# 86885974647565434342125458569795756674/torch.distributed.pipeline.sync.Pipe

Hardware: AMD Instinct MI355X
Metric: tokens/sec for 12-layer Transformer at PP=N (pipeline-parallel training) (higher is better)
Workload: dtype bf16

## Files before the change

mipipe/csrc/bindings.cpp:

```cpp
#include <torch/extension.h>
#include <ATen/hip/HIPContext.h>
#include <ATen/hip/HIPGeneratorImpl.h>
#include <ATen/core/Generator.h>
#include <ATen/hip/impl/HIPGuardImplMasqueradingAsCUDA.h>
#include <ATen/hip/impl/HIPStreamMasqueradingAsCUDA.h>

#include <mutex>
#include <optional>
#include <tuple>

#include "kernels/kernels.h"
#include "runtime/ipc.h"
#include "runtime/runtime.h"

namespace py = pybind11;
using at::Tensor;

namespace mipipe {
namespace {

#define MP_CHECK(cond, ...) TORCH_CHECK(cond, "mipipe: ", __VA_ARGS__)

hipStream_t cur_stream(const Tensor& t) { return at::hip::getCurrentHIPStreamMasqueradingAsCUDA(t.device().index()).stream(); }

// ... 1126 lines not shown
  m.def("attention_supported", [](int64_t S, int64_t D) { return attention_supported((int)S, (int)D); });
  m.def("attention_f32_supported", [](int64_t S, int64_t D) { return attention_f32_supported((int)S, (int)D); });
  m.def("attention_fwd", &py_attention_fwd, py::arg("q"), py::arg("k"), py::arg("v"), py::arg("causal"), py::arg("p"),
        py::arg("scale"), py::arg("kv_len") = 0, py::arg("words") = py::none(), py::arg("words_seed") = 0,
        py::arg("words_offset") = 0);
  m.def("attention_bwd", &py_attention_bwd, py::arg("dout"), py::arg("q"), py::arg("k"), py::arg("v"), py::arg("o"),
        py::arg("lse"), py::arg("causal"), py::arg("p"), py::arg("scale"), py::arg("seed"), py::arg("offset"),
        py::arg("dq"), py::arg("dk"), py::arg("dv"), py::arg("bits") = py::none(), py::arg("kv_len") = 0);
  m.def("attention_long_supported", [](int64_t S, int64_t D) { return attention_long_supported((int)S, (int)D); });
  m.def("attention_long_set_fused_rng", &attention_long_set_fused_rng,
        "long-sequence attention: make the dropout keep words inside the forward kernel (true, default) or in a "
        "kernel of their own before it (false)");
  m.def("gemm_supported", &py_gemm_supported);
  m.def("gemm_f32_supported", &py_gemm_f32_supported);
  m.def("attention_set_fused_bwd", &attention_set_fused_bwd);
  m.def("gemm_set_schedule", &gemm_set_schedule,
        "256x256 GEMM main loop: 7 whole-tile ping-pong (default, the only one in the product build); a "
        "--gemm-ab build also has the A/B schedules 0-6 (kernels.h).  Returns false for a schedule not built in.");
  m.def("gemm_get_schedule", &gemm_get_schedule);
  m.def("gemm_ab_build", &gemm_ab_build, "true if the A/B GEMM schedules 0-6 are compiled in (-DMIPIPE_GEMM_AB)");
  m.def("gemm_set_rounds", &gemm_set_rounds,
        "multi-round GEMM grids whose last round is at most half full: 0 one launch, 1 (default) one launch per round "
        "of tiles when K >= 4096, 2 one launch per round at any K");
  m.def("gemm_set_splitk", &gemm_set_splitk, "split-K factor of under-filled long-K GEMMs: 0 off, 1 auto (default), n >= 2 forced");
  m.def("gemm_set_waves", &gemm_set_waves,
        "256x256 GEMM blocks: 4 = one wave per SIMD with a 128x128 tile each (gemm4w_kernel), 8 = the ping-pong kernel, "
        "0 = default");
  m.def("gemm_get_waves", &gemm_get_waves);
  m.def("gemm_set_width", &gemm_set_width, "256-row GEMM block width: 0 auto (grid-quantisation rule), 128, 256");
  m.def("linear_fwd", &py_linear_fwd, py::arg("x"), py::arg("w"), py::arg("bias"), py::arg("act"), py::arg("p"),
// ... 29 lines not shown
```

mipipe/csrc/kernels/attention.hip:

```cpp
#include "common.h"
#include "kernels.h"

namespace mipipe {

namespace {

typedef __attribute__((ext_vector_type(4))) short s16x4;
typedef __attribute__((ext_vector_type(8))) short s16x8;
typedef __attribute__((address_space(3))) s16x4 lds_s16x4;

constexpr int kRows = 64;
constexpr int kThreads = 256;
constexpr float kLog2e = 1.4426950408889634f;

template <int D>
struct Img {
  static constexpr int kRowBytes = 2 * D;
  static constexpr int kChunks = D / 8;
  static constexpr int kBytes = kRows * kRowBytes;
  __device__ static __forceinline__ int f(int r) {
    if constexpr (kChunks >= 16) return (((r ^ (r >> 2)) & 1) << 1) | ((r & 2) << 1) | (r & 8);
    else if constexpr (kChunks == 8) return ((((r >> 1) ^ (r >> 2)) & 1) << 1) | ((r >> 1) & 4);
    else return (((r & 3) << 2) | ((r >> 2) & 3)) & (kChunks - 1);
  }
// ... 822 lines not shown
    }
}

namespace shortseq {

constexpr int S = 128;
constexpr int kThreads = 512;
constexpr int kChunk = 64;
constexpr int kChunkImg = S * kChunk * 2;
constexpr int kSqImg = S * S * 2;
constexpr int kStageBytes = 3 * kChunkImg;
constexpr int kPOff = 4 * kChunkImg;
constexpr int kDsOff = kPOff + kSqImg;
constexpr int kSmem = kDsOff + kSqImg;
constexpr int kFwdPOff = 2 * kChunkImg;
constexpr int kFwdSmem = kFwdPOff + kSqImg;

__device__ __forceinline__ int coff(int r, int c16) { return Img<64>::off(r, c16); }
__device__ __forceinline__ int soff(int r, int c16) { return Img<128>::off(r, c16); }

__device__ __forceinline__ void load_chunk(const bf16_t* __restrict__ base, int64_t ld, int d0, int tid, uint4& v0,
                                           uint4& v1) {
  const int r = tid >> 3, c = tid & 7;
  v0 = *reinterpret_cast<const uint4*>(base + (int64_t)r * ld + d0 + 8 * c);
  v1 = *reinterpret_cast<const uint4*>(base + (int64_t)(r + 64) * ld + d0 + 8 * c);
}
__device__ __forceinline__ void store_chunk(char* img, int tid, const uint4& v0, const uint4& v1) {
  const int r = tid >> 3, c = tid & 7;
  *reinterpret_cast<uint4*>(img + coff(r, c)) = v0;
  *reinterpret_cast<uint4*>(img + coff(r + 64, c)) = v1;
}

__device__ __forceinline__ bf16x8 crow(const char* img, int rb, int s, int lane) {
  return *reinterpret_cast<const bf16x8*>(img + coff(rb + (lane & 15), 4 * s + (lane >> 4)));
}
__device__ __forceinline__ bf16x8 ccol(const char* img, int db, int s, int lane) {
  const int g = lane >> 4, q = (lane & 15) >> 2, p = lane & 3;
  const int r0 = 32 * s + 8 * g + q;
  const int c8 = (db >> 2) + p;
  const int o0 = coff(r0, c8 >> 1) + 8 * (c8 & 1);
  const int o1 = coff(r0 + 4, c8 >> 1) + 8 * (c8 & 1);
  const s16x4 lo = __builtin_amdgcn_ds_read_tr16_b64_v4i16((lds_s16x4*)(img + o0));
  const s16x4 hi = __builtin_amdgcn_ds_read_tr16_b64_v4i16((lds_s16x4*)(img + o1));
  return __builtin_bit_cast(bf16x8, __builtin_shufflevector(lo, hi, 0, 1, 2, 3, 4, 5, 6, 7));
}
__device__ __forceinline__ bf16x8 srow(const char* img, int rb, int s, int lane) {
  return *reinterpret_cast<const bf16x8*>(img + soff(rb + (lane & 15), 4 * s + (lane >> 4)));
}
__device__ __forceinline__ bf16x8 scol(const char* img, int ib, int s, int lane) {
  const int g = lane >> 4, q = (lane & 15) >> 2, p = lane & 3;
  const int r0 = 32 * s + 8 * g + q;
  const int c8 = (ib >> 2) + p;
  const int o0 = soff(r0, c8 >> 1) + 8 * (c8 & 1);
  const int o1 = soff(r0 + 4, c8 >> 1) + 8 * (c8 & 1);
  const s16x4 lo = __builtin_amdgcn_ds_read_tr16_b64_v4i16((lds_s16x4*)(img + o0));
  const s16x4 hi = __builtin_amdgcn_ds_read_tr16_b64_v4i16((lds_s16x4*)(img + o1));
  return __builtin_bit_cast(bf16x8, __builtin_shufflevector(lo, hi, 0, 1, 2, 3, 4, 5, 6, 7));
}

template <int D, bool CAUSAL>
__global__ void __launch_bounds__(kThreads, 1) attn_bwd_s128_kernel(AttnArgs a) {
  extern __shared__ __attribute__((aligned(16))) char smem[];
  const int tid = threadIdx.x, lane = tid & 63, wave = __builtin_amdgcn_readfirstlane(tid >> 6);
  const int bh = blockIdx.x;
  const int b = bh / a.H, h = bh % a.H;
  const int64_t boff = (int64_t)b * a.sb_qkv + (int64_t)h * a.sh_qkv;
  const bf16_t* Q = reinterpret_cast<const bf16_t*>(a.q) + boff;
  const bf16_t* K = reinterpret_cast<const bf16_t*>(a.k) + boff;
  const bf16_t* V = reinterpret_cast<const bf16_t*>(a.v) + boff;
  const bf16_t* dO = reinterpret_cast<const bf16_t*>(a.dout) + (int64_t)b * a.sb_o + (int64_t)h * a.sh_o;
  constexpr int NC = D / kChunk;

  f32x4 sacc[8], pacc[8];
#pragma unroll
  for (int j = 0; j < 8; ++j) sacc[j] = pacc[j] = f32x4{0.f, 0.f, 0.f, 0.f};
  const int myrow = wave * 16 + (lane & 15);
  const bf16_t* qrow = Q + (int64_t)myrow * a.ld_qkv;
  const bf16_t* drow = dO + (int64_t)myrow * a.ld_o;

  uint4 k0, k1, v0, v1;
  load_chunk(K, a.ld_qkv, 0, tid, k0, k1);
  load_chunk(V, a.ld_qkv, 0, tid, v0, v1);
  store_chunk(smem, tid, k0, k1);
  store_chunk(smem + kChunkImg, tid, v0, v1);
  __syncthreads();
#pragma unroll 1
  for (int c = 0; c < NC; ++c) {
    const char* kimg = smem + (c & 1) * 2 * kChunkImg;
    const char* vimg = kimg + kChunkImg;
    if (c + 1 < NC) {
      load_chunk(K, a.ld_qkv, (c + 1) * kChunk, tid, k0, k1);
      load_chunk(V, a.ld_qkv, (c + 1) * kChunk, tid, v0, v1);
    }
    bf16x8 qf[2], df[2];
#pragma unroll
    for (int s2 = 0; s2 < 2; ++s2) {
      qf[s2] = frag_global(qrow + c * kChunk, s2, lane);
      df[s2] = frag_global(drow + c * kChunk, s2, lane);
    }
#pragma unroll
    for (int s2 = 0; s2 < 2; ++s2)
#pragma unroll
      for (int j = 0; j < 8; ++j) {
        sacc[j] = __builtin_amdgcn_mfma_f32_16x16x32_bf16(qf[s2], crow(kimg, 16 * j, s2, lane), sacc[j], 0, 0, 0);
        pacc[j] = __builtin_amdgcn_mfma_f32_16x16x32_bf16(df[s2], crow(vimg, 16 * j, s2, lane), pacc[j], 0, 0, 0);
      }
    if (c + 1 < NC) {
      char* nimg = smem + ((c + 1) & 1) * 2 * kChunkImg;
      store_chunk(nimg, tid, k0, k1);
      store_chunk(nimg + kChunkImg, tid, v0, v1);
    }
    __syncthreads();
  }

  const int qrow0 = wave * 16 + 4 * (lane >> 4);
  const float sl2 = a.scale * kLog2e;
  const float pscale = a.p > 0.f ? 1.f / (1.f - a.p) : 1.f;
  float lse2[4];
#pragma unroll
  for (int r = 0; r < 4; ++r) lse2[r] = a.lse[(int64_t)bh * S + qrow0 + r] * kLog2e;
  float dsum[4] = {0.f, 0.f, 0.f, 0.f};
#pragma unroll
  for (int j = 0; j < 8; ++j) {
    const int key = 16 * j + (lane & 15);
    uint32_t w[4] = {0xFFFFFFFFu, 0xFFFFFFFFu, 0xFFFFFFFFu, 0xFFFFFFFFu};
    if (a.p > 0.f) {
      const uint4 mw = attn_mask_words(a, bh, qrow0 >> 2, key);
      w[0] = mw.x; w[1] = mw.y; w[2] = mw.z; w[3] = mw.w;
    }
#pragma unroll
    for (int r = 0; r < 4; ++r) {
      float pr = __builtin_amdgcn_exp2f(sacc[j][r] * sl2 - lse2[r]);
      if (CAUSAL && key > qrow0 + r) pr = 0.f;
      float dp = pacc[j][r];
      float pd = pr;
      if (a.p > 0.f) {
        const bool keep = w[r] >= a.threshold;
        dp = keep ? dp * pscale : 0.f;
        pd = keep ? pr * pscale : 0.f;
      }
      sacc[j][r] = pr;
      pacc[j][r] = dp;
      dsum[r] += pr * dp;
      *reinterpret_cast<bf16_t*>(smem + kPOff + soff(qrow0 + r, key >> 3) + 2 * (key & 7)) = f2bf(pd);
    }
  }
  float delta[4];
#pragma unroll
  for (int r = 0; r < 4; ++r) delta[r] = row_reduce_sum16(dsum[r]);
#pragma unroll
  for (int j = 0; j < 8; ++j) {
    const int key = 16 * j + (lane & 15);
#pragma unroll
    for (int r = 0; r < 4; ++r) {
      const float ds = sacc[j][r] * (pacc[j][r] - delta[r]);
      *reinterpret_cast<bf16_t*>(smem + kDsOff + soff(qrow0 + r, key >> 3) + 2 * (key & 7)) = f2bf(ds);
    }
  }

  const char* pimg = smem + kPOff;
  const char* dsimg = smem + kDsOff;
  char* kimg = smem;
  char* qimg = smem + kChunkImg;
  char* dimg = smem + 2 * kChunkImg;
  bf16_t* dQ = reinterpret_cast<bf16_t*>(a.dq) + boff;
  bf16_t* dK = reinterpret_cast<bf16_t*>(a.dk) + boff;
  bf16_t* dV = reinterpret_cast<bf16_t*>(a.dv) + boff;
  const int r0 = wave * 16;
  uint4 a0, a1, b0, b1, e0, e1;
  load_chunk(K, a.ld_qkv, 0, tid, a0, a1);
  load_chunk(Q, a.ld_qkv, 0, tid, b0, b1);
  load_chunk(dO, a.ld_o, 0, tid, e0, e1);
#pragma unroll 1
  for (int c = 0; c < NC; ++c) {
    const int d0 = c * kChunk;
    __syncthreads();
    store_chunk(kimg, tid, a0, a1);
    store_chunk(qimg, tid, b0, b1);
    store_chunk(dimg, tid, e0, e1);
    __syncthreads();
    if (c + 1 < NC) {
      load_chunk(K, a.ld_qkv, d0 + kChunk, tid, a0, a1);
      load_chunk(Q, a.ld_qkv, d0 + kChunk, tid, b0, b1);
      load_chunk(dO, a.ld_o, d0 + kChunk, tid, e0, e1);
    }
    f32x4 dq[4], dk[4], dv[4];
#pragma unroll
    for (int t = 0; t < 4; ++t) dq[t] = dk[t] = dv[t] = f32x4{0.f, 0.f, 0.f, 0.f};
#pragma unroll
    for (int ks = 0; ks < 4; ++ks) {
      const bf16x8 a_dq = srow(dsimg, r0, ks, lane);
      const bf16x8 a_dk = scol(dsimg, r0, ks, lane);
      const bf16x8 a_dv = scol(pimg, r0, ks, lane);
#pragma unroll
      for (int t = 0; t < 4; ++t) {
        dq[t] = __builtin_amdgcn_mfma_f32_16x16x32_bf16(a_dq, ccol(kimg, 16 * t, ks, lane), dq[t], 0, 0, 0);
        dk[t] = __builtin_amdgcn_mfma_f32_16x16x32_bf16(a_dk, ccol(qimg, 16 * t, ks, lane), dk[t], 0, 0, 0);
        dv[t] = __builtin_amdgcn_mfma_f32_16x16x32_bf16(a_dv, ccol(dimg, 16 * t, ks, lane), dv[t], 0, 0, 0);
      }
    }
    const int orow = r0 + 4 * (lane >> 4);
    __syncthreads();
#pragma unroll
    for (int t = 0; t < 4; ++t) {
      const int col = 16 * t + (lane & 15);
#pragma unroll
      for (int r = 0; r < 4; ++r) {
        const int at = coff(orow + r, col >> 3) + 2 * (col & 7);
        *reinterpret_cast<bf16_t*>(kimg + at) = f2bf(dq[t][r] * a.scale);
        *reinterpret_cast<bf16_t*>(qimg + at) = f2bf(dk[t][r] * a.scale);
        *reinterpret_cast<bf16_t*>(dimg + at) = f2bf(dv[t][r]);
      }
    }
    __syncthreads();
    {
      const int r = tid >> 3, cc = tid & 7;
#pragma unroll
      for (int h2 = 0; h2 < 2; ++h2) {
        const int row = r + 64 * h2;
        const int off = coff(row, cc);
        const int64_t g = (int64_t)row * a.ld_qkv + d0 + 8 * cc;
        *reinterpret_cast<uint4*>(dQ + g) = *reinterpret_cast<const uint4*>(kimg + off);
        *reinterpret_cast<uint4*>(dK + g) = *reinterpret_cast<const uint4*>(qimg + off);
        *reinterpret_cast<uint4*>(dV + g) = *reinterpret_cast<const uint4*>(dimg + off);
      }
    }
  }
}

template <int D, bool CAUSAL>
__global__ void __launch_bounds__(kThreads, 2) attn_fwd_s128_kernel(AttnArgs a) {
  extern __shared__ __attribute__((aligned(16))) char smem[];
  const int tid = threadIdx.x, lane = tid & 63, wave = __builtin_amdgcn_readfirstlane(tid >> 6);
  const int bh = blockIdx.x;
  const int b = bh / a.H, h = bh % a.H;
  const int64_t boff = (int64_t)b * a.sb_qkv + (int64_t)h * a.sh_qkv;
  const bf16_t* Q = reinterpret_cast<const bf16_t*>(a.q) + boff;
  const bf16_t* K = reinterpret_cast<const bf16_t*>(a.k) + boff;
  const bf16_t* V = reinterpret_cast<const bf16_t*>(a.v) + boff;
  constexpr int NC = D / kChunk;

  f32x4 sacc[8];
#pragma unroll
  for (int j = 0; j < 8; ++j) sacc[j] = f32x4{0.f, 0.f, 0.f, 0.f};
  const bf16_t* qrow = Q + (int64_t)(wave * 16 + (lane & 15)) * a.ld_qkv;

  uint4 k0, k1;
  load_chunk(K, a.ld_qkv, 0, tid, k0, k1);
  store_chunk(smem, tid, k0, k1);
  __syncthreads();
#pragma unroll 1
  for (int c = 0; c < NC; ++c) {
    const char* kimg = smem + (c & 1) * kChunkImg;
    if (c + 1 < NC) load_chunk(K, a.ld_qkv, (c + 1) * kChunk, tid, k0, k1);
    bf16x8 qf[2];
#pragma unroll
    for (int s2 = 0; s2 < 2; ++s2) qf[s2] = frag_global(qrow + c * kChunk, s2, lane);
#pragma unroll
    for (int s2 = 0; s2 < 2; ++s2)
#pragma unroll
      for (int j = 0; j < 8; ++j)
        sacc[j] = __builtin_amdgcn_mfma_f32_16x16x32_bf16(qf[s2], crow(kimg, 16 * j, s2, lane), sacc[j], 0, 0, 0);
    if (c + 1 < NC) store_chunk(smem + ((c + 1) & 1) * kChunkImg, tid, k0, k1);
    __syncthreads();
  }

  const int qrow0 = wave * 16 + 4 * (lane >> 4);
  const float sl2 = a.scale * kLog2e;
  const float pscale = a.p > 0.f ? 1.f / (1.f - a.p) : 1.f;
  float mx[4] = {-INFINITY, -INFINITY, -INFINITY, -INFINITY};
#pragma unroll
  for (int j = 0; j < 8; ++j) {
    const int key = 16 * j + (lane & 15);
#pragma unroll
    for (int r = 0; r < 4; ++r) {
      float x = sacc[j][r] * sl2;
      if (CAUSAL && key > qrow0 + r) x = -INFINITY;
      sacc[j][r] = x;
      mx[r] = fmaxf(mx[r], x);
    }
  }
#pragma unroll
  for (int r = 0; r < 4; ++r) mx[r] = row_reduce_max16(mx[r]);
  float sum[4] = {0.f, 0.f, 0.f, 0.f};
#pragma unroll
  for (int j = 0; j < 8; ++j)
#pragma unroll
    for (int r = 0; r < 4; ++r) {
      const float e = __builtin_amdgcn_exp2f(sacc[j][r] - mx[r]);
      sacc[j][r] = e;
      sum[r] += e;
    }
  float inv[4];
#pragma unroll
  for (int r = 0; r < 4; ++r) {
    sum[r] = row_reduce_sum16(sum[r]);
    inv[r] = 1.f / sum[r];
  }
  char* pimg = smem + kFwdPOff;
#pragma unroll
  for (int j = 0; j < 8; ++j) {
    const int key = 16 * j + (lane & 15);
    uint32_t w[4] = {0xFFFFFFFFu, 0xFFFFFFFFu, 0xFFFFFFFFu, 0xFFFFFFFFu};
    if (a.p > 0.f) {
      const uint4 mw = attn_mask_words(a, bh, qrow0 >> 2, key);
      w[0] = mw.x; w[1] = mw.y; w[2] = mw.z; w[3] = mw.w;
    }
#pragma unroll
    for (int r = 0; r < 4; ++r) {
      float pv = sacc[j][r] * inv[r];
      if (a.p > 0.f) pv = w[r] >= a.threshold ? pv * pscale : 0.f;
      *reinterpret_cast<bf16_t*>(pimg + soff(qrow0 + r, key >> 3) + 2 * (key & 7)) = f2bf(pv);
    }
  }
  if ((lane & 15) == 0) {
#pragma unroll
    for (int r = 0; r < 4; ++r) a.lse[(int64_t)bh * S + qrow0 + r] = (mx[r] + log2f(sum[r])) / kLog2e;
  }

  bf16_t* O = reinterpret_cast<bf16_t*>(a.o) + (int64_t)b * a.sb_o + (int64_t)h * a.sh_o;
  uint4 v0, v1;
  load_chunk(V, a.ld_qkv, 0, tid, v0, v1);
  store_chunk(smem, tid, v0, v1);
  __syncthreads();
  const int r0 = wave * 16;
#pragma unroll 1
  for (int c = 0; c < NC; ++c) {
    const char* vimg = smem + (c & 1) * kChunkImg;
    if (c + 1 < NC) load_chunk(V, a.ld_qkv, (c + 1) * kChunk, tid, v0, v1);
    f32x4 o[4];
#pragma unroll
    for (int t = 0; t < 4; ++t) o[t] = f32x4{0.f, 0.f, 0.f, 0.f};
#pragma unroll
    for (int ks = 0; ks < 4; ++ks) {
      const bf16x8 ap = srow(pimg, r0, ks, lane);
#pragma unroll
      for (int t = 0; t < 4; ++t)
        o[t] = __builtin_amdgcn_mfma_f32_16x16x32_bf16(ap, ccol(vimg, 16 * t, ks, lane), o[t], 0, 0, 0);
    }
    const int orow = r0 + 4 * (lane >> 4);
#pragma unroll
    for (int t = 0; t < 4; ++t)
#pragma unroll
      for (int r = 0; r < 4; ++r)
        O[(int64_t)(orow + r) * a.ld_o + c * kChunk + 16 * t + (lane & 15)] = f2bf(o[t][r]);
    if (c + 1 < NC) store_chunk(smem + ((c + 1) & 1) * kChunkImg, tid, v0, v1);
    __syncthreads();
  }
}

}

template <int D>
size_t fwd_smem() { return 2 * Img<D>::kBytes + 4 * 16 * kScrStride * 2; }
template <int D>
size_t dkdv_smem() { return fwd_smem<D>() + 128 * sizeof(float); }

int g_attn_fused_bwd = 1;
const int g_attn_wide = [] {
  const char* e = getenv("MIPIPE_ATTN_WIDE");
  return e == nullptr ? 1 : atoi(e);
}();

template <typename Kern>
void set_smem(Kern k, size_t bytes) {
  hipFuncSetAttribute(reinterpret_cast<const void*>(k), hipFuncAttributeMaxDynamicSharedMemorySize, (int)bytes);
}

template <int D, bool CAUSAL>
void run_fwd(const AttnArgs& a, hipStream_t s) {
  if (a.S == shortseq::S && g_attn_fused_bwd) {
    static bool once_s = false;
    if (!once_s) {
      set_smem(shortseq::attn_fwd_s128_kernel<D, CAUSAL>, shortseq::kFwdSmem);
      once_s = true;
    }
    hipLaunchKernelGGL((shortseq::attn_fwd_s128_kernel<D, CAUSAL>), dim3(a.B * a.H), dim3(shortseq::kThreads),
                       shortseq::kFwdSmem, s, a);
    return;
  }
  if (D == 64 && a.S % kWideRows == 0 && g_attn_wide) {
    static bool once_w = false;
    if (!once_w) { set_smem(attn_fwd_wide_kernel<CAUSAL>, wide_fwd_smem()); once_w = true; }
    hipLaunchKernelGGL((attn_fwd_wide_kernel<CAUSAL>), dim3(a.S / kWideRows, a.B * a.H), dim3(kThreads),
                       wide_fwd_smem(), s, a);
    return;
  }
  const size_t sm = fwd_smem<D>();
  static bool once = false;
  if (!once) { set_smem(attn_fwd_kernel<D, CAUSAL>, sm); once = true; }
  hipLaunchKernelGGL((attn_fwd_kernel<D, CAUSAL>), dim3(a.S / kRows, a.B * a.H), dim3(kThreads), sm, s, a);
}

template <int D, bool CAUSAL>
void run_bwd(const AttnArgs& a, hipStream_t s) {
  const size_t sm = fwd_smem<D>(), sm2 = dkdv_smem<D>();
  static bool once = false;
  if (!once) {
    set_smem(attn_dq_kernel<D, CAUSAL>, sm);
    set_smem(attn_dkdv_kernel<D, CAUSAL>, sm2);
    once = true;
  }
  if (a.S == shortseq::S && g_attn_fused_bwd) {
    static bool once_s = false;
    if (!once_s) {
      set_smem(shortseq::attn_bwd_s128_kernel<D, CAUSAL>, shortseq::kSmem);
      once_s = true;
    }
    hipLaunchKernelGGL((shortseq::attn_bwd_s128_kernel<D, CAUSAL>), dim3(a.B * a.H), dim3(shortseq::kThreads),
                       shortseq::kSmem, s, a);
    return;
  }
  const int64_t rows = (int64_t)a.B * a.S * a.H;
  hipLaunchKernelGGL(attn_delta_kernel, dim3((unsigned)((rows + 3) / 4)), dim3(256), 0, s, a, D);
  hipLaunchKernelGGL((attn_dkdv_kernel<D, CAUSAL>), dim3(a.S / kRows, a.B * a.H), dim3(kThreads), sm2, s, a);
  if (D == 64 && a.S % kWideRows == 0 && g_attn_wide) {
    static bool once_w = false;
    if (!once_w) { set_smem(attn_dq_wide_kernel<CAUSAL>, wide_fwd_smem()); once_w = true; }
    hipLaunchKernelGGL((attn_dq_wide_kernel<CAUSAL>), dim3(a.S / kWideRows, a.B * a.H), dim3(kThreads),
                       wide_fwd_smem(), s, a);
    return;
  }
  hipLaunchKernelGGL((attn_dq_kernel<D, CAUSAL>), dim3(a.S / kRows, a.B * a.H), dim3(kThreads), sm, s, a);
}

}

void attention_set_fused_bwd(int on) { g_attn_fused_bwd = on; }

bool attention_supported(int S, int D) { return S > 0 && S % kRows == 0 && (D == 64 || D == 128 || D == 256); }

void attention_fwd(const AttnArgs& ai, hipStream_t s) {
  AttnArgs a = ai;
  a.threshold = dropout_threshold(a.p);
  if (a.causal) {
    if (a.D == 64) run_fwd<64, true>(a, s);
    else if (a.D == 128) run_fwd<128, true>(a, s);
    else run_fwd<256, true>(a, s);
  } else {
    if (a.D == 64) run_fwd<64, false>(a, s);
    else if (a.D == 128) run_fwd<128, false>(a, s);
    else run_fwd<256, false>(a, s);
  }
// ... 18 lines not shown
```

mipipe/csrc/kernels/kernels.h:

```cpp
#pragma once

#include <hip/hip_runtime.h>
#include <stdint.h>

namespace mipipe {

typedef uint16_t bf16_t;

template <typename T>
struct LnArgs {
  const T* x = nullptr;
  const T* res = nullptr;
  const T* gamma = nullptr;
  const T* beta = nullptr;
  T* y = nullptr;
  T* z = nullptr;
  float* mean = nullptr;
  float* rstd = nullptr;
  int rows = 0, cols = 0;
  float eps = 1e-5f;
  float p = 0.f;
  uint64_t seed = 0, offset = 0;
};

// ... 123 lines not shown
  float* lse = nullptr;
  float* delta = nullptr;
  int64_t ld_qkv = 0, ld_o = 0;
  int64_t sb_qkv = 0, sh_qkv = 0;
  int64_t sb_o = 0, sh_o = 0;
  int B = 0, H = 0, S = 0, D = 0;
  float scale = 1.f, p = 0.f;
  uint32_t threshold = 0;
  uint64_t seed = 0, offset = 0;
  bool causal = false;
  int kv_len = 0;
  uint32_t* dmask = nullptr;
};
bool attention_supported(int S, int D);
void attention_set_fused_bwd(int on);
void attention_fwd(const AttnArgs& a, hipStream_t s);
void attention_bwd(const AttnArgs& a, hipStream_t s);
bool attention_f32_supported(int S, int D);
bool attention_long_supported(int S, int D);
void attention_long_set_fused_rng(bool on);
void attention_long_fwd(const AttnArgs& a, hipStream_t s);
void attention_long_fwd_words(const AttnArgs& a, hipStream_t s);
void attention_long_bwd(const AttnArgs& a, hipStream_t s);
void attention_f32_fwd(const AttnArgs& a, hipStream_t s);
void attention_f32_bwd(const AttnArgs& a, hipStream_t s);

template <typename T>
void cross_entropy_fwd(const T* logits, const int64_t* target, int64_t rows, int64_t V, int64_t ld,
                       int64_t ignore_index, float* loss, float* lse, hipStream_t s, int64_t t_offset = 0);
template <typename T>
// ... 43 lines not shown
```

Measured before the change: 147,500.

## Make S=128 attention kernels persistent with cross-head prefetch and staged output stores

The S=128 forward and backward attention kernels now loop over several (batch, head) pairs per block. Each block prefetches the next head's K/V/Q/dO fragments during the current head's final chunk, and Q/dO fragments are register double-buffered across chunks. The backward grid is capped at one block per CU by default, and forward output goes through a per-wave LDS tile for coalesced 16-byte stores. This aims to hide global-load latency and launch tail effects, at the cost of extra LDS, more register pressure and less parallelism when there are few heads.

```diff
diff --git a/mipipe/csrc/bindings.cpp b/mipipe/csrc/bindings.cpp
--- a/mipipe/csrc/bindings.cpp
+++ b/mipipe/csrc/bindings.cpp
@@ -1164,6 +1164,8 @@
   m.def("gemm_supported", &py_gemm_supported);
   m.def("gemm_f32_supported", &py_gemm_f32_supported);
   m.def("attention_set_fused_bwd", &attention_set_fused_bwd);
+  m.def("attention_set_s128_grid", &attention_set_s128_grid, py::arg("fwd_blocks"), py::arg("bwd_blocks"),
+        "S = 128 attention kernels: blocks per launch (0 = default); each block walks several heads");
   m.def("gemm_set_schedule", &gemm_set_schedule,
         "256x256 GEMM main loop: 7 whole-tile ping-pong (default, the only one in the product build); a "
         "--gemm-ab build also has the A/B schedules 0-6 (kernels.h).  Returns false for a schedule not built in.");
diff --git a/mipipe/csrc/kernels/attention.hip b/mipipe/csrc/kernels/attention.hip
--- a/mipipe/csrc/kernels/attention.hip
+++ b/mipipe/csrc/kernels/attention.hip
@@ -860,7 +860,9 @@
 constexpr int kDsOff = kPOff + kSqImg;
 constexpr int kSmem = kDsOff + kSqImg;
 constexpr int kFwdPOff = 2 * kChunkImg;
-constexpr int kFwdSmem = kFwdPOff + kSqImg;
+constexpr int kFwdOOff = kFwdPOff + kSqImg;
+constexpr int kFwdOTile = 16 * kChunk * 2;
+constexpr int kFwdSmem = kFwdOOff + (kThreads / 64) * kFwdOTile;
 
 __device__ __forceinline__ int coff(int r, int c16) { return Img<64>::off(r, c16); }
 __device__ __forceinline__ int soff(int r, int c16) { return Img<128>::off(r, c16); }
@@ -878,7 +880,7 @@
 }
 
 __device__ __forceinline__ bf16x8 crow(const char* img, int rb, int s, int lane) {
-  return *reinterpret_cast<const bf16x8*>(img + coff(rb + (lane & 15), 4 * s + (lane >> 4)));
+  return *reinterpret_cast<const bf16x8*>(img + rb * (2 * kChunk) + coff(lane & 15, 4 * s + (lane >> 4)));
 }
 __device__ __forceinline__ bf16x8 ccol(const char* img, int db, int s, int lane) {
   const int g = lane >> 4, q = (lane & 15) >> 2, p = lane & 3;
@@ -908,169 +910,217 @@
 __global__ void __launch_bounds__(kThreads, 1) attn_bwd_s128_kernel(AttnArgs a) {
   extern __shared__ __attribute__((aligned(16))) char smem[];
   const int tid = threadIdx.x, lane = tid & 63, wave = __builtin_amdgcn_readfirstlane(tid >> 6);
-  const int bh = blockIdx.x;
-  const int b = bh / a.H, h = bh % a.H;
-  const int64_t boff = (int64_t)b * a.sb_qkv + (int64_t)h * a.sh_qkv;
-  const bf16_t* Q = reinterpret_cast<const bf16_t*>(a.q) + boff;
-  const bf16_t* K = reinterpret_cast<const bf16_t*>(a.k) + boff;
-  const bf16_t* V = reinterpret_cast<const bf16_t*>(a.v) + boff;
-  const bf16_t* dO = reinterpret_cast<const bf16_t*>(a.dout) + (int64_t)b * a.sb_o + (int64_t)h * a.sh_o;
   constexpr int NC = D / kChunk;
-
-  f32x4 sacc[8], pacc[8];
-#pragma unroll
-  for (int j = 0; j < 8; ++j) sacc[j] = pacc[j] = f32x4{0.f, 0.f, 0.f, 0.f};
+  const int nbh = a.B * a.H;
+  int bh = blockIdx.x;
+  if (bh >= nbh) return;
   const int myrow = wave * 16 + (lane & 15);
-  const bf16_t* qrow = Q + (int64_t)myrow * a.ld_qkv;
-  const bf16_t* drow = dO + (int64_t)myrow * a.ld_o;
 
   uint4 k0, k1, v0, v1;
-  load_chunk(K, a.ld_qkv, 0, tid, k0, k1);
-  load_chunk(V, a.ld_qkv, 0, tid, v0, v1);
-  store_chunk(smem, tid, k0, k1);
-  store_chunk(smem + kChunkImg, tid, v0, v1);
-  __syncthreads();
+  bf16x8 qn[2], dn[2];
+  {
+    const int b = bh / a.H, h = bh % a.H;
+    const int64_t boff = (int64_t)b * a.sb_qkv + (int64_t)h * a.sh_qkv;
+    const int64_t ooff = (int64_t)b * a.sb_o + (int64_t)h * a.sh_o;
+    const bf16_t* qr = reinterpret_cast<const bf16_t*>(a.q) + boff + (int64_t)myrow * a.ld_qkv;
+    const bf16_t* dr = reinterpret_cast<const bf16_t*>(a.dout) + ooff + (int64_t)myrow * a.ld_o;
+    load_chunk(reinterpret_cast<const bf16_t*>(a.k) + boff, a.ld_qkv, 0, tid, k0, k1);
+    load_chunk(reinterpret_cast<const bf16_t*>(a.v) + boff, a.ld_qkv, 0, tid, v0, v1);
+#pragma unroll
+    for (int s2 = 0; s2 < 2; ++s2) {
+      qn[s2] = frag_global(qr, s2, lane);
+      dn[s2] = frag_global(dr, s2, lane);
+    }
+  }
 #pragma unroll 1
-  for (int c = 0; c < NC; ++c) {
-    const char* kimg = smem + (c & 1) * 2 * kChunkImg;
-    const char* vimg = kimg + kChunkImg;
-    if (c + 1 < NC) {
-      load_chunk(K, a.ld_qkv, (c + 1) * kChunk, tid, k0, k1);
-      load_chunk(V, a.ld_qkv, (c + 1) * kChunk, tid, v0, v1);
-    }
-    bf16x8 qf[2], df[2];
-#pragma unroll
-    for (int s2 = 0; s2 < 2; ++s2) {
-      qf[s2] = frag_global(qrow + c * kChunk, s2, lane);
-      df[s2] = frag_global(drow + c * kChunk, s2, lane);
-    }
-#pragma unroll
-    for (int s2 = 0; s2 < 2; ++s2)
-#pragma unroll
-      for (int j = 0; j < 8; ++j) {
-        sacc[j] = __builtin_amdgcn_mfma_f32_16x16x32_bf16(qf[s2], crow(kimg, 16 * j, s2, lane), sacc[j], 0, 0, 0);
-        pacc[j] = __builtin_amdgcn_mfma_f32_16x16x32_bf16(df[s2], crow(vimg, 16 * j, s2, lane), pacc[j], 0, 0, 0);
-      }
-    if (c + 1 < NC) {
-      char* nimg = smem + ((c + 1) & 1) * 2 * kChunkImg;
-      store_chunk(nimg, tid, k0, k1);
-      store_chunk(nimg + kChunkImg, tid, v0, v1);
-    }
+  for (; bh < nbh; bh += gridDim.x) {
+    int tid_h = threadIdx.x;
+    asm volatile("" : "+v"(tid_h));
+    const int tid = tid_h, lane = tid & 63, wave = __builtin_amdgcn_readfirstlane(tid >> 6);
+    const int myrow = wave * 16 + (lane & 15);
+    const int b = bh / a.H, h = bh % a.H;
+    const int64_t boff = (int64_t)b * a.sb_qkv + (int64_t)h * a.sh_qkv;
+    const bf16_t* Q = reinterpret_cast<const bf16_t*>(a.q) + boff;
+    const bf16_t* K = reinterpret_cast<const bf16_t*>(a.k) + boff;
+    const bf16_t* V = reinterpret_cast<const bf16_t*>(a.v) + boff;
+    const bf16_t* dO = reinterpret_cast<const bf16_t*>(a.dout) + (int64_t)b * a.sb_o + (int64_t)h * a.sh_o;
+
+    f32x4 sacc[8], pacc[8];
+#pragma unroll
+    for (int j = 0; j < 8; ++j) sacc[j] = pacc[j] = f32x4{0.f, 0.f, 0.f, 0.f};
+    const bf16_t* qrow = Q + (int64_t)myrow * a.ld_qkv;
+    const bf16_t* drow = dO + (int64_t)myrow * a.ld_o;
+
+    store_chunk(smem, tid, k0, k1);
+    store_chunk(smem + kChunkImg, tid, v0, v1);
     __syncthreads();
-  }
-
-  const int qrow0 = wave * 16 + 4 * (lane >> 4);
-  const float sl2 = a.scale * kLog2e;
-  const float pscale = a.p > 0.f ? 1.f / (1.f - a.p) : 1.f;
-  float lse2[4];
-#pragma unroll
-  for (int r = 0; r < 4; ++r) lse2[r] = a.lse[(int64_t)bh * S + qrow0 + r] * kLog2e;
-  float dsum[4] = {0.f, 0.f, 0.f, 0.f};
-#pragma unroll
-  for (int j = 0; j < 8; ++j) {
-    const int key = 16 * j + (lane & 15);
-    uint32_t w[4] = {0xFFFFFFFFu, 0xFFFFFFFFu, 0xFFFFFFFFu, 0xFFFFFFFFu};
-    if (a.p > 0.f) {
-      const uint4 mw = attn_mask_words(a, bh, qrow0 >> 2, key);
-      w[0] = mw.x; w[1] = mw.y; w[2] = mw.z; w[3] = mw.w;
-    }
-#pragma unroll
-    for (int r = 0; r < 4; ++r) {
-      float pr = __builtin_amdgcn_exp2f(sacc[j][r] * sl2 - lse2[r]);
-      if (CAUSAL && key > qrow0 + r) pr = 0.f;
-      float dp = pacc[j][r];
-      float pd = pr;
+#pragma unroll
+    for (int c = 0; c < NC; ++c) {
+      const char* kimg = smem + (c & 1) * 2 * kChunkImg;
+      const char* vimg = kimg + kChunkImg;
+      bf16x8 qf[2], df[2];
+#pragma unroll
+      for (int s2 = 0; s2 < 2; ++s2) {
+        qf[s2] = qn[s2];
+        df[s2] = dn[s2];
+      }
+      if (c + 1 < NC) {
+#pragma unroll
+        for (int s2 = 0; s2 < 2; ++s2) {
+          qn[s2] = frag_global(qrow + (c + 1) * kChunk, s2, lane);
+          dn[s2] = frag_global(drow + (c + 1) * kChunk, s2, lane);
+        }
+        load_chunk(K, a.ld_qkv, (c + 1) * kChunk, tid, k0, k1);
+        load_chunk(V, a.ld_qkv, (c + 1) * kChunk, tid, v0, v1);
+      }
+      __builtin_amdgcn_sched_barrier(0);
+#pragma unroll
+      for (int s2 = 0; s2 < 2; ++s2)
+#pragma unroll
+        for (int j = 0; j < 8; ++j) {
+          sacc[j] = __builtin_amdgcn_mfma_f32_16x16x32_bf16(qf[s2], crow(kimg, 16 * j, s2, lane), sacc[j], 0, 0, 0);
+          pacc[j] = __builtin_amdgcn_mfma_f32_16x16x32_bf16(df[s2], crow(vimg, 16 * j, s2, lane), pacc[j], 0, 0, 0);
+        }
+      if (c + 1 < NC) {
+        char* nimg = smem + ((c + 1) & 1) * 2 * kChunkImg;
+        store_chunk(nimg, tid, k0, k1);
+        store_chunk(nimg + kChunkImg, tid, v0, v1);
+      }
+      __syncthreads();
+    }
+
+    const int qrow0 = wave * 16 + 4 * (lane >> 4);
+    float lse2[4];
+#pragma unroll
+    for (int r = 0; r < 4; ++r) lse2[r] = a.lse[(int64_t)bh * S + qrow0 + r];
+    uint4 a0, a1, b0, b1, e0, e1;
+    load_chunk(K, a.ld_qkv, 0, tid, a0, a1);
+    load_chunk(Q, a.ld_qkv, 0, tid, b0, b1);
+    load_chunk(dO, a.ld_o, 0, tid, e0, e1);
+
+    const float sl2 = a.scale * kLog2e;
+    const float pscale = a.p > 0.f ? 1.f / (1.f - a.p) : 1.f;
+#pragma unroll
+    for (int r = 0; r < 4; ++r) lse2[r] *= kLog2e;
+    float dsum[4] = {0.f, 0.f, 0.f, 0.f};
+#pragma unroll
+    for (int j = 0; j < 8; ++j) {
+      const int key = 16 * j + (lane & 15);
+      uint32_t w[4] = {0xFFFFFFFFu, 0xFFFFFFFFu, 0xFFFFFFFFu, 0xFFFFFFFFu};
       if (a.p > 0.f) {
-        const bool keep = w[r] >= a.threshold;
-        dp = keep ? dp * pscale : 0.f;
-        pd = keep ? pr * pscale : 0.f;
-      }
-      sacc[j][r] = pr;
-      pacc[j][r] = dp;
-      dsum[r] += pr * dp;
-      *reinterpret_cast<bf16_t*>(smem + kPOff + soff(qrow0 + r, key >> 3) + 2 * (key & 7)) = f2bf(pd);
-    }
-  }
-  float delta[4];
-#pragma unroll
-  for (int r = 0; r < 4; ++r) delta[r] = row_reduce_sum16(dsum[r]);
-#pragma unroll
-  for (int j = 0; j < 8; ++j) {
-    const int key = 16 * j + (lane & 15);
-#pragma unroll
-    for (int r = 0; r < 4; ++r) {
-      const float ds = sacc[j][r] * (pacc[j][r] - delta[r]);
-      *reinterpret_cast<bf16_t*>(smem + kDsOff + soff(qrow0 + r, key >> 3) + 2 * (key & 7)) = f2bf(ds);
-    }
-  }
-
-  const char* pimg = smem + kPOff;
-  const char* dsimg = smem + kDsOff;
-  char* kimg = smem;
-  char* qimg = smem + kChunkImg;
-  char* dimg = smem + 2 * kChunkImg;
-  bf16_t* dQ = reinterpret_cast<bf16_t*>(a.dq) + boff;
-  bf16_t* dK = reinterpret_cast<bf16_t*>(a.dk) + boff;
-  bf16_t* dV = reinterpret_cast<bf16_t*>(a.dv) + boff;
-  const int r0 = wave * 16;
-  uint4 a0, a1, b0, b1, e0, e1;
-  load_chunk(K, a.ld_qkv, 0, tid, a0, a1);
-  load_chunk(Q, a.ld_qkv, 0, tid, b0, b1);
-  load_chunk(dO, a.ld_o, 0, tid, e0, e1);
-#pragma unroll 1
-  for (int c = 0; c < NC; ++c) {
-    const int d0 = c * kChunk;
+        const uint4 mw = attn_mask_words(a, bh, qrow0 >> 2, key);
+        w[0] = mw.x; w[1] = mw.y; w[2] = mw.z; w[3] = mw.w;
+      }
+#pragma unroll
+      for (int r = 0; r < 4; ++r) {
+        float pr = __builtin_amdgcn_exp2f(sacc[j][r] * sl2 - lse2[r]);
+        if (CAUSAL && key > qrow0 + r) pr = 0.f;
+        float dp = pacc[j][r];
+        float pd = pr;
+        if (a.p > 0.f) {
+          const bool keep = w[r] >= a.threshold;
+          dp = keep ? dp * pscale : 0.f;
+          pd = keep ? pr * pscale : 0.f;
+        }
+        sacc[j][r] = pr;
+        pacc[j][r] = dp;
+        dsum[r] += pr * dp;
+        *reinterpret_cast<bf16_t*>(smem + kPOff + soff(qrow0 + r, key >> 3) + 2 * (key & 7)) = f2bf(pd);
+      }
+    }
+    float delta[4];
+#pragma unroll
+    for (int r = 0; r < 4; ++r) delta[r] = row_reduce_sum16(dsum[r]);
+#pragma unroll
+    for (int j = 0; j < 8; ++j) {
+      const int key = 16 * j + (lane & 15);
+#pragma unroll
+      for (int r = 0; r < 4; ++r) {
+        const float ds = sacc[j][r] * (pacc[j][r] - delta[r]);
+        *reinterpret_cast<bf16_t*>(smem + kDsOff + soff(qrow0 + r, key >> 3) + 2 * (key & 7)) = f2bf(ds);
+      }
+    }
+
+    const char* pimg = smem + kPOff;
+    const char* dsimg = smem + kDsOff;
+    char* kimg = smem;
+    char* qimg = smem + kChunkImg;
+    char* dimg = smem + 2 * kChunkImg;
+    bf16_t* dQ = reinterpret_cast<bf16_t*>(a.dq) + boff;
+    bf16_t* dK = reinterpret_cast<bf16_t*>(a.dk) + boff;
+    bf16_t* dV = reinterpret_cast<bf16_t*>(a.dv) + boff;
+    const int r0 = wave * 16;
+    const bool more = bh + (int)gridDim.x < nbh;
+#pragma unroll
+    for (int c = 0; c < NC; ++c) {
+      const int d0 = c * kChunk;
+      __syncthreads();
+      store_chunk(kimg, tid, a0, a1);
+      store_chunk(qimg, tid, b0, b1);
+      store_chunk(dimg, tid, e0, e1);
+      __syncthreads();
+      if (c + 1 < NC) {
+        load_chunk(K, a.ld_qkv, d0 + kChunk, tid, a0, a1);
+        load_chunk(Q, a.ld_qkv, d0 + kChunk, tid, b0, b1);
+        load_chunk(dO, a.ld_o, d0 + kChunk, tid, e0, e1);
+      } else if (more) {
+        const int nb = (bh + (int)gridDim.x) / a.H, nh = (bh + (int)gridDim.x) % a.H;
+        const int64_t noff = (int64_t)nb * a.sb_qkv + (int64_t)nh * a.sh_qkv;
+        const int64_t nooff = (int64_t)nb * a.sb_o + (int64_t)nh * a.sh_o;
+        const bf16_t* qr = reinterpret_cast<const bf16_t*>(a.q) + noff + (int64_t)myrow * a.ld_qkv;
+        const bf16_t* dr = reinterpret_cast<const bf16_t*>(a.dout) + nooff + (int64_t)myrow * a.ld_o;
+        load_chunk(reinterpret_cast<const bf16_t*>(a.k) + noff, a.ld_qkv, 0, tid, k0, k1);
+        load_chunk(reinterpret_cast<const bf16_t*>(a.v) + noff, a.ld_qkv, 0, tid, v0, v1);
+#pragma unroll
+        for (int s2 = 0; s2 < 2; ++s2) {
+          qn[s2] = frag_global(qr, s2, lane);
+          dn[s2] = frag_global(dr, s2, lane);
+        }
+      }
+      __builtin_amdgcn_sched_barrier(0);
+      f32x4 dq[4], dk[4], dv[4];
+#pragma unroll
+      for (int t = 0; t < 4; ++t) dq[t] = dk[t] = dv[t] = f32x4{0.f, 0.f, 0.f, 0.f};
+#pragma unroll
+      for (int ks = 0; ks < 4; ++ks) {
+        const bf16x8 a_dq = srow(dsimg, r0, ks, lane);
+        const bf16x8 a_dk = scol(dsimg, r0, ks, lane);
+        const bf16x8 a_dv = scol(pimg, r0, ks, lane);
+#pragma unroll
+        for (int t = 0; t < 4; ++t) {
+          dq[t] = __builtin_amdgcn_mfma_f32_16x16x32_bf16(a_dq, ccol(kimg, 16 * t, ks, lane), dq[t], 0, 0, 0);
+          dk[t] = __builtin_amdgcn_mfma_f32_16x16x32_bf16(a_dk, ccol(qimg, 16 * t, ks, lane), dk[t], 0, 0, 0);
+          dv[t] = __builtin_amdgcn_mfma_f32_16x16x32_bf16(a_dv, ccol(dimg, 16 * t, ks, lane), dv[t], 0, 0, 0);
+        }
+      }
+      const int orow = r0 + 4 * (lane >> 4);
+      __syncthreads();
+#pragma unroll
+      for (int t = 0; t < 4; ++t) {
+        const int col = 16 * t + (lane & 15);
+#pragma unroll
+        for (int r = 0; r < 4; ++r) {
+          const int at = coff(orow + r, col >> 3) + 2 * (col & 7);
+          *reinterpret_cast<bf16_t*>(kimg + at) = f2bf(dq[t][r] * a.scale);
+          *reinterpret_cast<bf16_t*>(qimg + at) = f2bf(dk[t][r] * a.scale);
+          *reinterpret_cast<bf16_t*>(dimg + at) = f2bf(dv[t][r]);
+        }
+      }
+      __syncthreads();
+      {
+        const int r = tid >> 3, cc = tid & 7;
+#pragma unroll
+        for (int h2 = 0; h2 < 2; ++h2) {
+          const int row = r + 64 * h2;
+          const int off = coff(row, cc);
+          const int64_t g = (int64_t)row * a.ld_qkv + d0 + 8 * cc;
+          *reinterpret_cast<uint4*>(dQ + g) = *reinterpret_cast<const uint4*>(kimg + off);
+          *reinterpret_cast<uint4*>(dK + g) = *reinterpret_cast<const uint4*>(qimg + off);
+          *reinterpret_cast<uint4*>(dV + g) = *reinterpret_cast<const uint4*>(dimg + off);
+        }
+      }
+    }
     __syncthreads();
-    store_chunk(kimg, tid, a0, a1);
-    store_chunk(qimg, tid, b0, b1);
-    store_chunk(dimg, tid, e0, e1);
-    __syncthreads();
-    if (c + 1 < NC) {
-      load_chunk(K, a.ld_qkv, d0 + kChunk, tid, a0, a1);
-      load_chunk(Q, a.ld_qkv, d0 + kChunk, tid, b0, b1);
-      load_chunk(dO, a.ld_o, d0 + kChunk, tid, e0, e1);
-    }
-    f32x4 dq[4], dk[4], dv[4];
-#pragma unroll
-    for (int t = 0; t < 4; ++t) dq[t] = dk[t] = dv[t] = f32x4{0.f, 0.f, 0.f, 0.f};
-#pragma unroll
-    for (int ks = 0; ks < 4; ++ks) {
-      const bf16x8 a_dq = srow(dsimg, r0, ks, lane);
-      const bf16x8 a_dk = scol(dsimg, r0, ks, lane);
-      const bf16x8 a_dv = scol(pimg, r0, ks, lane);
-#pragma unroll
-      for (int t = 0; t < 4; ++t) {
-        dq[t] = __builtin_amdgcn_mfma_f32_16x16x32_bf16(a_dq, ccol(kimg, 16 * t, ks, lane), dq[t], 0, 0, 0);
-        dk[t] = __builtin_amdgcn_mfma_f32_16x16x32_bf16(a_dk, ccol(qimg, 16 * t, ks, lane), dk[t], 0, 0, 0);
-        dv[t] = __builtin_amdgcn_mfma_f32_16x16x32_bf16(a_dv, ccol(dimg, 16 * t, ks, lane), dv[t], 0, 0, 0);
-      }
-    }
-    const int orow = r0 + 4 * (lane >> 4);
-    __syncthreads();
-#pragma unroll
-    for (int t = 0; t < 4; ++t) {
-      const int col = 16 * t + (lane & 15);
-#pragma unroll
-      for (int r = 0; r < 4; ++r) {
-        const int at = coff(orow + r, col >> 3) + 2 * (col & 7);
-        *reinterpret_cast<bf16_t*>(kimg + at) = f2bf(dq[t][r] * a.scale);
-        *reinterpret_cast<bf16_t*>(qimg + at) = f2bf(dk[t][r] * a.scale);
-        *reinterpret_cast<bf16_t*>(dimg + at) = f2bf(dv[t][r]);
-      }
-    }
-    __syncthreads();
-    {
-      const int r = tid >> 3, cc = tid & 7;
-#pragma unroll
-      for (int h2 = 0; h2 < 2; ++h2) {
-        const int row = r + 64 * h2;
-        const int off = coff(row, cc);
-        const int64_t g = (int64_t)row * a.ld_qkv + d0 + 8 * cc;
-        *reinterpret_cast<uint4*>(dQ + g) = *reinterpret_cast<const uint4*>(kimg + off);
-        *reinterpret_cast<uint4*>(dK + g) = *reinterpret_cast<const uint4*>(qimg + off);
-        *reinterpret_cast<uint4*>(dV + g) = *reinterpret_cast<const uint4*>(dimg + off);
-      }
-    }
   }
 }
 
@@ -1078,120 +1128,164 @@
 __global__ void __launch_bounds__(kThreads, 2) attn_fwd_s128_kernel(AttnArgs a) {
   extern __shared__ __attribute__((aligned(16))) char smem[];
   const int tid = threadIdx.x, lane = tid & 63, wave = __builtin_amdgcn_readfirstlane(tid >> 6);
-  const int bh = blockIdx.x;
-  const int b = bh / a.H, h = bh % a.H;
-  const int64_t boff = (int64_t)b * a.sb_qkv + (int64_t)h * a.sh_qkv;
-  const bf16_t* Q = reinterpret_cast<const bf16_t*>(a.q) + boff;
-  const bf16_t* K = reinterpret_cast<const bf16_t*>(a.k) + boff;
-  const bf16_t* V = reinterpret_cast<const bf16_t*>(a.v) + boff;
   constexpr int NC = D / kChunk;
-
-  f32x4 sacc[8];
-#pragma unroll
-  for (int j = 0; j < 8; ++j) sacc[j] = f32x4{0.f, 0.f, 0.f, 0.f};
-  const bf16_t* qrow = Q + (int64_t)(wave * 16 + (lane & 15)) * a.ld_qkv;
+  const int nbh = a.B * a.H;
+  int bh = blockIdx.x;
+  if (bh >= nbh) return;
+  const int myrow = wave * 16 + (lane & 15);
 
   uint4 k0, k1;
-  load_chunk(K, a.ld_qkv, 0, tid, k0, k1);
-  store_chunk(smem, tid, k0, k1);
-  __syncthreads();
+  bf16x8 qn[2];
+  {
+    const int64_t boff = (int64_t)(bh / a.H) * a.sb_qkv + (int64_t)(bh % a.H) * a.sh_qkv;
+    const bf16_t* qr = reinterpret_cast<const bf16_t*>(a.q) + boff + (int64_t)myrow * a.ld_qkv;
+    load_chunk(reinterpret_cast<const bf16_t*>(a.k) + boff, a.ld_qkv, 0, tid, k0, k1);
+#pragma unroll
+    for (int s2 = 0; s2 < 2; ++s2) qn[s2] = frag_global(qr, s2, lane);
+  }
 #pragma unroll 1
-  for (int c = 0; c < NC; ++c) {
-    const char* kimg = smem + (c & 1) * kChunkImg;
-    if (c + 1 < NC) load_chunk(K, a.ld_qkv, (c + 1) * kChunk, tid, k0, k1);
-    bf16x8 qf[2];
-#pragma unroll
-    for (int s2 = 0; s2 < 2; ++s2) qf[s2] = frag_global(qrow + c * kChunk, s2, lane);
-#pragma unroll
-    for (int s2 = 0; s2 < 2; ++s2)
-#pragma unroll
-      for (int j = 0; j < 8; ++j)
-        sacc[j] = __builtin_amdgcn_mfma_f32_16x16x32_bf16(qf[s2], crow(kimg, 16 * j, s2, lane), sacc[j], 0, 0, 0);
-    if (c + 1 < NC) store_chunk(smem + ((c + 1) & 1) * kChunkImg, tid, k0, k1);
+  for (; bh < nbh; bh += gridDim.x) {
+    int tid_h = threadIdx.x;
+    asm volatile("" : "+v"(tid_h));
+    const int tid = tid_h, lane = tid & 63, wave = __builtin_amdgcn_readfirstlane(tid >> 6);
+    const int myrow = wave * 16 + (lane & 15);
+    const int b = bh / a.H, h = bh % a.H;
+    const int64_t boff = (int64_t)b * a.sb_qkv + (int64_t)h * a.sh_qkv;
+    const bf16_t* Q = reinterpret_cast<const bf16_t*>(a.q) + boff;
+    const bf16_t* K = reinterpret_cast<const bf16_t*>(a.k) + boff;
+    const bf16_t* V = reinterpret_cast<const bf16_t*>(a.v) + boff;
+
+    f32x4 sacc[8];
+#pragma unroll
+    for (int j = 0; j < 8; ++j) sacc[j] = f32x4{0.f, 0.f, 0.f, 0.f};
+    const bf16_t* qrow = Q + (int64_t)myrow * a.ld_qkv;
+
+    store_chunk(smem, tid, k0, k1);
     __syncthreads();
-  }
-
-  const int qrow0 = wave * 16 + 4 * (lane >> 4);
-  const float sl2 = a.scale * kLog2e;
-  const float pscale = a.p > 0.f ? 1.f / (1.f - a.p) : 1.f;
-  float mx[4] = {-INFINITY, -INFINITY, -INFINITY, -INFINITY};
-#pragma unroll
-  for (int j = 0; j < 8; ++j) {
-    const int key = 16 * j + (lane & 15);
+#pragma unroll
+    for (int c = 0; c < NC; ++c) {
+      const char* kimg = smem + (c & 1) * kChunkImg;
+      bf16x8 qf[2];
+#pragma unroll
+      for (int s2 = 0; s2 < 2; ++s2) qf[s2] = qn[s2];
+      if (c + 1 < NC) {
+#pragma unroll
+        for (int s2 = 0; s2 < 2; ++s2) qn[s2] = frag_global(qrow + (c + 1) * kChunk, s2, lane);
+        load_chunk(K, a.ld_qkv, (c + 1) * kChunk, tid, k0, k1);
+      }
+      __builtin_amdgcn_sched_barrier(0);
+#pragma unroll
+      for (int s2 = 0; s2 < 2; ++s2)
+#pragma unroll
+        for (int j = 0; j < 8; ++j)
+          sacc[j] = __builtin_amdgcn_mfma_f32_16x16x32_bf16(qf[s2], crow(kimg, 16 * j, s2, lane), sacc[j], 0, 0, 0);
+      if (c + 1 < NC) store_chunk(smem + ((c + 1) & 1) * kChunkImg, tid, k0, k1);
+      __syncthreads();
+    }
+
+    uint4 v0, v1;
+    load_chunk(V, a.ld_qkv, 0, tid, v0, v1);
+
+    const int qrow0 = wave * 16 + 4 * (lane >> 4);
+    const float sl2 = a.scale * kLog2e;
+    const float pscale = a.p > 0.f ? 1.f / (1.f - a.p) : 1.f;
+    float mx[4] = {-INFINITY, -INFINITY, -INFINITY, -INFINITY};
+#pragma unroll
+    for (int j = 0; j < 8; ++j) {
+      const int key = 16 * j + (lane & 15);
+#pragma unroll
+      for (int r = 0; r < 4; ++r) {
+        float x = sacc[j][r] * sl2;
+        if (CAUSAL && key > qrow0 + r) x = -INFINITY;
+        sacc[j][r] = x;
+        mx[r] = fmaxf(mx[r], x);
+      }
+    }
+#pragma unroll
+    for (int r = 0; r < 4; ++r) mx[r] = row_reduce_max16(mx[r]);
+    float sum[4] = {0.f, 0.f, 0.f, 0.f};
+#pragma unroll
+    for (int j = 0; j < 8; ++j)
+#pragma unroll
+      for (int r = 0; r < 4; ++r) {
+        const float e = __builtin_amdgcn_exp2f(sacc[j][r] - mx[r]);
+        sacc[j][r] = e;
+        sum[r] += e;
+      }
+    float inv[4];
 #pragma unroll
     for (int r = 0; r < 4; ++r) {
-      float x = sacc[j][r] * sl2;
-      if (CAUSAL && key > qrow0 + r) x = -INFINITY;
-      sacc[j][r] = x;
-      mx[r] = fmaxf(mx[r], x);
-    }
-  }
-#pragma unroll
-  for (int r = 0; r < 4; ++r) mx[r] = row_reduce_max16(mx[r]);
-  float sum[4] = {0.f, 0.f, 0.f, 0.f};
-#pragma unroll
-  for (int j = 0; j < 8; ++j)
-#pragma unroll
-    for (int r = 0; r < 4; ++r) {
-      const float e = __builtin_amdgcn_exp2f(sacc[j][r] - mx[r]);
-      sacc[j][r] = e;
-      sum[r] += e;
-    }
-  float inv[4];
-#pragma unroll
-  for (int r = 0; r < 4; ++r) {
-    sum[r] = row_reduce_sum16(sum[r]);
-    inv[r] = 1.f / sum[r];
-  }
-  char* pimg = smem + kFwdPOff;
-#pragma unroll
-  for (int j = 0; j < 8; ++j) {
-    const int key = 16 * j + (lane & 15);
-    uint32_t w[4] = {0xFFFFFFFFu, 0xFFFFFFFFu, 0xFFFFFFFFu, 0xFFFFFFFFu};
-    if (a.p > 0.f) {
-      const uint4 mw = attn_mask_words(a, bh, qrow0 >> 2, key);
-      w[0] = mw.x; w[1] = mw.y; w[2] = mw.z; w[3] = mw.w;
-    }
-#pragma unroll
-    for (int r = 0; r < 4; ++r) {
-      float pv = sacc[j][r] * inv[r];
-      if (a.p > 0.f) pv = w[r] >= a.threshold ? pv * pscale : 0.f;
-      *reinterpret_cast<bf16_t*>(pimg + soff(qrow0 + r, key >> 3) + 2 * (key & 7)) = f2bf(pv);
-    }
-  }
-  if ((lane & 15) == 0) {
-#pragma unroll
-    for (int r = 0; r < 4; ++r) a.lse[(int64_t)bh * S + qrow0 + r] = (mx[r] + log2f(sum[r])) / kLog2e;
-  }
-
-  bf16_t* O = reinterpret_cast<bf16_t*>(a.o) + (int64_t)b * a.sb_o + (int64_t)h * a.sh_o;
-  uint4 v0, v1;
-  load_chunk(V, a.ld_qkv, 0, tid, v0, v1);
-  store_chunk(smem, tid, v0, v1);
-  __syncthreads();
-  const int r0 = wave * 16;
-#pragma unroll 1
-  for (int c = 0; c < NC; ++c) {
-    const char* vimg = smem + (c & 1) * kChunkImg;
-    if (c + 1 < NC) load_chunk(V, a.ld_qkv, (c + 1) * kChunk, tid, v0, v1);
-    f32x4 o[4];
-#pragma unroll
-    for (int t = 0; t < 4; ++t) o[t] = f32x4{0.f, 0.f, 0.f, 0.f};
-#pragma unroll
-    for (int ks = 0; ks < 4; ++ks) {
-      const bf16x8 ap = srow(pimg, r0, ks, lane);
-#pragma unroll
-      for (int t = 0; t < 4; ++t)
-        o[t] = __builtin_amdgcn_mfma_f32_16x16x32_bf16(ap, ccol(vimg, 16 * t, ks, lane), o[t], 0, 0, 0);
-    }
-    const int orow = r0 + 4 * (lane >> 4);
-#pragma unroll
-    for (int t = 0; t < 4; ++t)
-#pragma unroll
-      for (int r = 0; r < 4; ++r)
-        O[(int64_t)(orow + r) * a.ld_o + c * kChunk + 16 * t + (lane & 15)] = f2bf(o[t][r]);
-    if (c + 1 < NC) store_chunk(smem + ((c + 1) & 1) * kChunkImg, tid, v0, v1);
+      sum[r] = row_reduce_sum16(sum[r]);
+      inv[r] = 1.f / sum[r];
+    }
+    store_chunk(smem, tid, v0, v1);
+    char* pimg = smem + kFwdPOff;
+#pragma unroll
+    for (int j = 0; j < 8; ++j) {
+      const int key = 16 * j + (lane & 15);
+      uint32_t w[4] = {0xFFFFFFFFu, 0xFFFFFFFFu, 0xFFFFFFFFu, 0xFFFFFFFFu};
+      if (a.p > 0.f) {
+        const uint4 mw = attn_mask_words(a, bh, qrow0 >> 2, key);
+        w[0] = mw.x; w[1] = mw.y; w[2] = mw.z; w[3] = mw.w;
+      }
+#pragma unroll
+      for (int r = 0; r < 4; ++r) {
+        float pv = sacc[j][r] * inv[r];
+        if (a.p > 0.f) pv = w[r] >= a.threshold ? pv * pscale : 0.f;
+        *reinterpret_cast<bf16_t*>(pimg + soff(qrow0 + r, key >> 3) + 2 * (key & 7)) = f2bf(pv);
+      }
+    }
+    if ((lane & 15) == 0) {
+#pragma unroll
+      for (int r = 0; r < 4; ++r) a.lse[(int64_t)bh * S + qrow0 + r] = (mx[r] + log2f(sum[r])) / kLog2e;
+    }
+
+    bf16_t* O = reinterpret_cast<bf16_t*>(a.o) + (int64_t)b * a.sb_o + (int64_t)h * a.sh_o;
     __syncthreads();
+    const int r0 = wave * 16;
+    char* ot = smem + kFwdOOff + wave * kFwdOTile;
+    const bool more = bh + (int)gridDim.x < nbh;
+    const int nbh1 = more ? bh + (int)gridDim.x : bh;
+    const int64_t noff = (int64_t)(nbh1 / a.H) * a.sb_qkv + (int64_t)(nbh1 % a.H) * a.sh_qkv;
+#pragma unroll
+    for (int c = 0; c < NC; ++c) {
+      const char* vimg = smem + (c & 1) * kChunkImg;
+      if (c + 1 < NC) {
+        load_chunk(V, a.ld_qkv, (c + 1) * kChunk, tid, v0, v1);
+      } else if (more) {
+        const bf16_t* qr = reinterpret_cast<const bf16_t*>(a.q) + noff + (int64_t)myrow * a.ld_qkv;
+        load_chunk(reinterpret_cast<const bf16_t*>(a.k) + noff, a.ld_qkv, 0, tid, k0, k1);
+#pragma unroll
+        for (int s2 = 0; s2 < 2; ++s2) qn[s2] = frag_global(qr, s2, lane);
+      }
+      __builtin_amdgcn_sched_barrier(0);
+      f32x4 o[4];
+#pragma unroll
+      for (int t = 0; t < 4; ++t) o[t] = f32x4{0.f, 0.f, 0.f, 0.f};
+#pragma unroll
+      for (int ks = 0; ks < 4; ++ks) {
+        const bf16x8 ap = srow(pimg, r0, ks, lane);
+#pragma unroll
+        for (int t = 0; t < 4; ++t)
+          o[t] = __builtin_amdgcn_mfma_f32_16x16x32_bf16(ap, ccol(vimg, 16 * t, ks, lane), o[t], 0, 0, 0);
+      }
+#pragma unroll
+      for (int t = 0; t < 4; ++t) {
+        const int col = 16 * t + (lane & 15);
+#pragma unroll
+        for (int r = 0; r < 4; ++r)
+          *reinterpret_cast<bf16_t*>(ot + coff(4 * (lane >> 4) + r, col >> 3) + 2 * (col & 7)) = f2bf(o[t][r]);
+      }
+      __builtin_amdgcn_s_waitcnt(0xC07F);
+#pragma unroll
+      for (int h2 = 0; h2 < 2; ++h2) {
+        const int row = (lane >> 3) + 8 * h2, cc = lane & 7;
+        *reinterpret_cast<uint4*>(O + (int64_t)(r0 + row) * a.ld_o + c * kChunk + 8 * cc) =
+            *reinterpret_cast<const uint4*>(ot + coff(row, cc));
+      }
+      if (c + 1 < NC) store_chunk(smem + ((c + 1) & 1) * kChunkImg, tid, v0, v1);
+      __syncthreads();
+    }
   }
 }
 
@@ -1207,6 +1301,29 @@
   const char* e = getenv("MIPIPE_ATTN_WIDE");
   return e == nullptr ? 1 : atoi(e);
 }();
+
+int g_s128_fwd_blocks = 0, g_s128_bwd_blocks = 0;
+constexpr int kS128FwdPerCu = 0, kS128BwdPerCu = 1;
+
+int cu_count() {
+  constexpr int kMaxDev = 64;
+  static int cus[kMaxDev] = {};
+  int dev = 0;
+  if (hipGetDevice(&dev) != hipSuccess || dev < 0 || dev >= kMaxDev) return 0;
+  if (cus[dev] == 0) {
+    hipDeviceProp_t prop;
+    if (hipGetDeviceProperties(&prop, dev) != hipSuccess) return 0;
+    cus[dev] = prop.multiProcessorCount;
+  }
+  return cus[dev];
+}
+
+int s128_grid(int forced, int per_cu, const AttnArgs& a) {
+  const int heads = a.B * a.H;
+  if (forced > 0) return forced;
+  const int resident = per_cu * cu_count();
+  return resident <= 0 || heads < resident ? heads : resident;
+}
 
 template <typename Kern>
 void set_smem(Kern k, size_t bytes) {
@@ -1221,8 +1338,8 @@
       set_smem(shortseq::attn_fwd_s128_kernel<D, CAUSAL>, shortseq::kFwdSmem);
       once_s = true;
     }
-    hipLaunchKernelGGL((shortseq::attn_fwd_s128_kernel<D, CAUSAL>), dim3(a.B * a.H), dim3(shortseq::kThreads),
-                       shortseq::kFwdSmem, s, a);
+    hipLaunchKernelGGL((shortseq::attn_fwd_s128_kernel<D, CAUSAL>), dim3(s128_grid(g_s128_fwd_blocks, kS128FwdPerCu, a)),
+                       dim3(shortseq::kThreads), shortseq::kFwdSmem, s, a);
     return;
   }
   if (D == 64 && a.S % kWideRows == 0 && g_attn_wide) {
@@ -1253,8 +1370,8 @@
       set_smem(shortseq::attn_bwd_s128_kernel<D, CAUSAL>, shortseq::kSmem);
       once_s = true;
     }
-    hipLaunchKernelGGL((shortseq::attn_bwd_s128_kernel<D, CAUSAL>), dim3(a.B * a.H), dim3(shortseq::kThreads),
-                       shortseq::kSmem, s, a);
+    hipLaunchKernelGGL((shortseq::attn_bwd_s128_kernel<D, CAUSAL>), dim3(s128_grid(g_s128_bwd_blocks, kS128BwdPerCu, a)),
+                       dim3(shortseq::kThreads), shortseq::kSmem, s, a);
     return;
   }
   const int64_t rows = (int64_t)a.B * a.S * a.H;
@@ -1273,6 +1390,11 @@
 }
 
 void attention_set_fused_bwd(int on) { g_attn_fused_bwd = on; }
+
+void attention_set_s128_grid(int fwd_blocks, int bwd_blocks) {
+  g_s128_fwd_blocks = fwd_blocks > 0 ? fwd_blocks : 0;
+  g_s128_bwd_blocks = bwd_blocks > 0 ? bwd_blocks : 0;
+}
 
 bool attention_supported(int S, int D) { return S > 0 && S % kRows == 0 && (D == 64 || D == 128 || D == 256); }
 
diff --git a/mipipe/csrc/kernels/kernels.h b/mipipe/csrc/kernels/kernels.h
--- a/mipipe/csrc/kernels/kernels.h
+++ b/mipipe/csrc/kernels/kernels.h
@@ -161,6 +161,7 @@
 };
 bool attention_supported(int S, int D);
 void attention_set_fused_bwd(int on);
+void attention_set_s128_grid(int fwd_blocks, int bwd_blocks);
 void attention_fwd(const AttnArgs& a, hipStream_t s);
 void attention_bwd(const AttnArgs& a, hipStream_t s);
 bool attention_f32_supported(int S, int D);
```

Result: no change. 147,900 (median of 6 runs) (+0.3%).
